# olivier-2018/scene_3Dreconstruction_MVSNet

Measured on AMD Instinct MI355X. Metric: depth maps/sec at N=5 views, 640x512, D=192; achieved HBM GB/s, higher is better.
Workload: dtype f32 (conv0, conv2-4, conv9, conv11: 3xbf16 split operands on the bf16 matrix cores, fp32 accumulate)

## Files before the change

### scene_3dreconstruction_mvsnet_amd/csrc/conv3d_mfma16.hip

```cpp
#include <cstdlib>
#include <cstring>

#include "mvs_internal.h"
#include "storage.h"
#include "mfma16_ops.h"

namespace mvs {

typedef unsigned short u16x8 __attribute__((ext_vector_type(8)));

static inline uint16_t to_bits16(float v, int dt) {
    uint16_t out;
    if (dt == MVS_F16) {
        const _Float16 h = (_Float16)v;
        std::memcpy(&out, &h, 2);
    } else {
        uint32_t u;
        std::memcpy(&u, &v, 4);
        if ((u & 0x7F800000u) == 0x7F800000u && (u & 0x007FFFFFu)) return (uint16_t)((u >> 16) | 0x0040u);
        u += 0x7FFFu + ((u >> 16) & 1u);
        out = (uint16_t)(u >> 16);
    }
    return out;
}

template <int DT>
struct Op16 {
    using T = unsigned short;
    static constexpr int NPC = 1;
    static constexpr bool CLAMP = false;
    struct Stage {
        u32x4 v;
        __device__ __forceinline__ void load(const T* plane, int goff) { v = *reinterpret_cast<const u32x4*>(plane + goff); }
        __device__ __forceinline__ void stage(unsigned short* tile, int tile_elems, int loff, bool inside) const {
            if (loff >= 0) *reinterpret_cast<u32x4*>(tile + loff) = inside ? v : (u32x4){0u, 0u, 0u, 0u};
        }
    };
    template <int N>
    static __device__ __forceinline__ void mac(f32x4& acc, const unsigned short* ap, int tile_elems, const u32x4 (&b)[N], int ks) {
        acc = mfma16<DT>(*reinterpret_cast<const u32x4*>(ap), b[ks], acc);
    }
    struct Skip { float v[8]; };
    static __device__ __forceinline__ void load8(const T* p, size_t idx, Skip& s) { load8_16<DT>(p, idx, s.v); }
    static __device__ __forceinline__ void store8(T* p, size_t idx, f32x4 lo, f32x4 hi) {
        const float v[8] = {lo.x, lo.y, lo.z, lo.w, hi.x, hi.y, hi.z, hi.w};
        store8_16<DT>(p, idx, v);
    }
    static __device__ __forceinline__ void store8(T* p, size_t idx, f32x4 lo, f32x4 hi, const Skip& s) {
        const float v[8] = {lo.x + s.v[0], lo.y + s.v[1], lo.z + s.v[2], lo.w + s.v[3],
                            hi.x + s.v[4], hi.y + s.v[5], hi.z + s.v[6], hi.w + s.v[7]};
        store8_16<DT>(p, idx, v);
    }
};

struct OpSplit {
    using T = float;
    static constexpr int NPC = 3;
    static constexpr bool CLAMP = true;
    struct Stage {
        f32x4 lo, hi;
        __device__ __forceinline__ void load(const T* plane, int goff) {
            lo = *reinterpret_cast<const f32x4*>(plane + goff);
            hi = *reinterpret_cast<const f32x4*>(plane + goff + 4);
        }
        __device__ __forceinline__ void stage(unsigned short* tile, int tile_elems, int loff, bool inside) const {
            const f32x4 z4 = (f32x4){0.f, 0.f, 0.f, 0.f};
            u32x4 p1, p2, p3;
            gs_split8(inside ? lo : z4, inside ? hi : z4, p1, p2, p3);
            *reinterpret_cast<u32x4*>(tile + loff) = p1;
            *reinterpret_cast<u32x4*>(tile + tile_elems + loff) = p2;
            *reinterpret_cast<u32x4*>(tile + 2 * tile_elems + loff) = p3;
        }
    };
    template <int N>
    static __device__ __forceinline__ void mac(f32x4& acc, const unsigned short* ap, int tile_elems, const u32x4 (&b)[N], int ks) {
        constexpr int KS = N / NPC;
        const u32x4 a1 = *reinterpret_cast<const u32x4*>(ap);
        const u32x4 a2 = *reinterpret_cast<const u32x4*>(ap + tile_elems);
        const u32x4 a3 = *reinterpret_cast<const u32x4*>(ap + 2 * tile_elems);
        acc = mfma16<MVS_BF16>(a3, b[ks], acc);
        acc = mfma16<MVS_BF16>(a1, b[2 * KS + ks], acc);
        acc = mfma16<MVS_BF16>(a2, b[KS + ks], acc);
        acc = mfma16<MVS_BF16>(a2, b[ks], acc);
        acc = mfma16<MVS_BF16>(a1, b[KS + ks], acc);
        acc = mfma16<MVS_BF16>(a1, b[ks], acc);
    }
    struct Skip { f32x4 lo, hi; };
    static __device__ __forceinline__ void load8(const T* p, size_t idx, Skip& s) {
        s.lo = *reinterpret_cast<const f32x4*>(p + idx);
        s.hi = *reinterpret_cast<const f32x4*>(p + idx + 4);
    }
    static __device__ __forceinline__ void store8(T* p, size_t idx, f32x4 lo, f32x4 hi) {
        *reinterpret_cast<f32x4*>(p + idx) = lo;
        *reinterpret_cast<f32x4*>(p + idx + 4) = hi;
    }
    static __device__ __forceinline__ void store8(T* p, size_t idx, f32x4 lo, f32x4 hi, const Skip& s) {
        *reinterpret_cast<f32x4*>(p + idx) = lo + s.lo;
        *reinterpret_cast<f32x4*>(p + idx + 4) = hi + s.hi;
    }
};

template <int CIN, int COUT, int S, int BZ, int BY, int BX>
struct ConvG16 {
    static constexpr int NT = COUT / 16;
    static constexpr int MG = 4 / NT;
    static constexpr int MT = BZ * BY * BX;
    static constexpr int MPW = MT / MG;
    static constexpr int NCH = CIN / 8;
    static constexpr int KS = 7;
    static constexpr int VS = 8;
    static constexpr int HZ = (BZ - 1) * S + 3, HY = (2 * BY - 1) * S + 3, HX = (8 * BX - 1) * S + 3;
    static constexpr int HXP = ((HX + 7) / 8 * 8) | 8;
    static constexpr int TILE_ELEMS = HZ * HY * HXP * VS;
    static constexpr int NPIECE = HZ * HY * HX;
    static constexpr int PPT = (NPIECE + 255) / 256;
    static_assert(NT == 1 || NT == 2 || NT == 4, "COUT must be 16, 32 or 64");
    static_assert(MT % MG == 0, "block tile must split evenly over the M-groups");
    static_assert(PPT <= 32, "piece mask is 32 bits");
    static constexpr int tap_off(int tap) {
        const int t = tap > 26 ? 26 : tap;
        return (((t / 9) * HY + (t / 3) % 3) * HXP + t % 3) * VS;
    }
};

template <class Op, int CIN, int COUT, int S, int BZ, int BY, int BX>
__global__ __launch_bounds__(256) void convg16_mfma_kernel(
    const typename Op::T* __restrict__ x,
    const unsigned short* __restrict__ bp,
    const float* __restrict__ bias,
    typename Op::T* __restrict__ y,
    int Di, int Hi, int Wi, int Do, int Ho, int Wo) {
    using G = ConvG16<CIN, COUT, S, BZ, BY, BX>;
    constexpr int OY = 2 * BY, OX = 8 * BX;
    constexpr int RP0 = OX * COUT + 16 * (OX / 8), RP = (RP0 % 32 == 16) ? RP0 : RP0 + 16;
    constexpr int OUT_FLOATS = BZ * OY * RP, NUNIT = BZ * OY * OX * (COUT / 8), UPT = (NUNIT + 255) / 256;
    constexpr int TILE_BYTES = Op::NPC * G::TILE_ELEMS * 2;
    constexpr int LDS_BYTES = TILE_BYTES > OUT_FLOATS * 4 ? TILE_BYTES : OUT_FLOATS * 4;
    __shared__ __attribute__((aligned(16))) unsigned char lds_raw[LDS_BYTES];
    unsigned short* tile = reinterpret_cast<unsigned short*>(lds_raw);
    float* otile = reinterpret_cast<float*>(lds_raw);

    const int tid = threadIdx.x, lane = tid & 63, wave = tid >> 6;
    const int nt = wave % G::NT, mg = wave / G::NT;
    const int nbx = (Wo + 8 * BX - 1) / (8 * BX), nby = (Ho + 2 * BY - 1) / (2 * BY);
    int b = xcd_block();
    const int bx = b % nbx; b /= nbx;
    const int by = b % nby;
    const int bz = b / nby;
    const int ox0 = bx * 8 * BX, oy0 = by * 2 * BY, oz0 = bz * BZ;
    const int ix0 = ox0 * S - 1, iy0 = oy0 * S - 1, iz0 = oz0 * S - 1;
    const size_t Vin = (size_t)Di * Hi * Wi, Vout = (size_t)Do * Ho * Wo;
    constexpr size_t PANEL = (size_t)G::NCH * G::NT * G::KS * 64;

    int goff[G::PPT], loff[G::PPT];
    unsigned inside = 0;
#pragma unroll
    for (int i = 0; i < G::PPT; ++i) {
        const int v = Op::CLAMP ? min(tid + i * 256, G::NPIECE - 1) : tid + i * 256;
        const int hx = v % G::HX, t = v / G::HX;
        const int hy = t % G::HY, hz = t / G::HY;
        const int gz = iz0 + hz, gy = iy0 + hy, gx = ix0 + hx;
        const bool live = Op::CLAMP || v < G::NPIECE;
        const bool ok = live && gz >= 0 && gz < Di && gy >= 0 && gy < Hi && gx >= 0 && gx < Wi;
        goff[i] = ok ? (int)((((size_t)gz * Hi + gy) * Wi + gx) * 8) : 0;
        inside |= ok ? (1u << i) : 0u;
        loff[i] = live ? ((hz * G::HY + hy) * G::HXP + hx) * G::VS : -1;
    }

    const int r = lane & 15, g = lane >> 4;
    const int ry = r >> 3, rx = r & 7;
    int abase[G::MPW];
#pragma unroll
    for (int i = 0; i < G::MPW; ++i) {
        const int t = mg * G::MPW + i;
        const int tx = t % BX, ty = (t / BX) % BY, tz = t / (BX * BY);
        abase[i] = (((tz * S) * G::HY + (2 * ty + ry) * S) * G::HXP + (8 * tx + rx) * S) * G::VS;
    }
    int koff[G::KS];
#pragma unroll
    for (int ks = 0; ks < G::KS; ++ks)
        koff[ks] = g == 0 ? G::tap_off(4 * ks) : g == 1 ? G::tap_off(4 * ks + 1)
                 : g == 2 ? G::tap_off(4 * ks + 2) : G::tap_off(4 * ks + 3);

    f32x4 acc[G::MPW];
#pragma unroll
    for (int i = 0; i < G::MPW; ++i) acc[i] = (f32x4){0.f, 0.f, 0.f, 0.f};
    u32x4 breg[Op::NPC * G::KS];
    typename Op::Stage stg[G::PPT];

    auto load_b = [&](int c) {
        const u32x4* bsrc = reinterpret_cast<const u32x4*>(bp) + ((size_t)(c * G::NT + nt) * G::KS) * 64 + lane;
#pragma unroll
        for (int q = 0; q < Op::NPC; ++q)
#pragma unroll
            for (int ks = 0; ks < G::KS; ++ks) breg[q * G::KS + ks] = bsrc[q * PANEL + ks * 64];
    };
    auto load_a = [&](int c) {
        const typename Op::T* plane = x + (size_t)c * Vin * 8;
#pragma unroll
        for (int i = 0; i < G::PPT; ++i) stg[i].load(plane, goff[i]);
    };
    auto store_a = [&]() {
#pragma unroll
        for (int i = 0; i < G::PPT; ++i) stg[i].stage(tile, G::TILE_ELEMS, loff[i], (inside >> i) & 1u);
    };

    load_b(0);
    load_a(0);
    store_a();
    __syncthreads();

#pragma unroll 1
    for (int c = 0; c < G::NCH; ++c) {
        if (c + 1 < G::NCH) load_a(c + 1);
#pragma unroll
        for (int ks = 0; ks < G::KS; ++ks) {
#pragma unroll
            for (int i = 0; i < G::MPW; ++i) Op::mac(acc[i], tile + abase[i] + koff[ks], G::TILE_ELEMS, breg, ks);
        }
        if (c + 1 < G::NCH) {
            load_b(c + 1);
            __syncthreads();
            store_a();
            __syncthreads();
        }
    }

    const int n = lane & 15, co = 16 * nt + n;
    const float bv = bias[co];
    __syncthreads();
#pragma unroll
    for (int i = 0; i < G::MPW; ++i) {
        const int t = mg * G::MPW + i;
        const int tx = t % BX, ty = (t / BX) % BY, tz = t / (BX * BY);
#pragma unroll
        for (int e = 0; e < 4; ++e) {
            const int m = 4 * (lane >> 4) + e;
            const int oy = 2 * ty + (m >> 3), ox = 8 * tx + (m & 7);
            otile[(tz * OY + oy) * RP + ox * COUT + (ox >> 3) * 16 + co] = relu(acc[i][e] + bv);
        }
    }
    __syncthreads();
#pragma unroll
    for (int j = 0; j < UPT; ++j) {
        const int u = tid + j * 256;
        const int ox = u % OX;
        int t = u / OX;
        const int oy = t % OY; t /= OY;
        const int ozl = t % BZ, pl = t / BZ;
        const int gz = oz0 + ozl, gy = oy0 + oy, gx = ox0 + ox;
        if (u < NUNIT && gz < Do && gy < Ho && gx < Wo) {
            const float* src = otile + (ozl * OY + oy) * RP + ox * COUT + (ox >> 3) * 16 + pl * 8;
            const f32x4 lo = *reinterpret_cast<const f32x4*>(src), hi = *reinterpret_cast<const f32x4*>(src + 4);
            Op::store8(y, ((size_t)pl * Vout + ((size_t)gz * Ho + gy) * Wo + gx) * 8, lo, hi);
        }
    }
}

template <class Op, int CIN, int COUT, int S, int BZ, int BY, int BX>
static int run_convg16(const void* x, void* y, const unsigned short* bp, const float* bias, int Di, int Hi,
                       int Wi, hipStream_t s) {
    using T = typename Op::T;
    const int Do = (Di - 1) / S + 1, Ho = (Hi - 1) / S + 1, Wo = (Wi - 1) / S + 1;
    if ((size_t)Di * Hi * Wi * 8 >= ((size_t)1 << 31))
        return fail(MVS_ERR_BAD_SHAPE, "convg16_mfma: plane exceeds 31-bit offsets");
    const int nb = ((Wo + 8 * BX - 1) / (8 * BX)) * ((Ho + 2 * BY - 1) / (2 * BY)) * ((Do + BZ - 1) / BZ);
    convg16_mfma_kernel<Op, CIN, COUT, S, BZ, BY, BX><<<nb, 256, 0, s>>>(static_cast<const T*>(x), bp, bias,
                                                                         static_cast<T*>(y), Di, Hi, Wi, Do, Ho, Wo);
    return check_hip(hipGetLastError(), "convg16_mfma launch");
}

static bool tile_fills_chip(int Di, int Hi, int Wi, int S, int BZ, int BY, int BX) {
    const int force = options().deep_tiles;
    if (force >= 0) return force != 0;
    const int cus = device_cus();
    const int Do = (Di - 1) / S + 1, Ho = (Hi - 1) / S + 1, Wo = (Wi - 1) / S + 1;
    const long nb = (long)((Wo + 8 * BX - 1) / (8 * BX)) * ((Ho + 2 * BY - 1) / (2 * BY)) * ((Do + BZ - 1) / BZ);
    return 2 * nb >= 3 * (long)cus;
}

template <int DT>
static int launch_convg16_dt(int layer, const void* x, void* y, const unsigned short* bp, const float* bias,
                             int Di, int Hi, int Wi, hipStream_t s) {
    switch (layer) {
        case 1: return run_convg16<Op16<DT>, 8, 16, 2, 2, 2, 2>(x, y, bp, bias, Di, Hi, Wi, s);
        case 2: return run_convg16<Op16<DT>, 16, 16, 1, 2, 4, 2>(x, y, bp, bias, Di, Hi, Wi, s);
        case 3: return run_convg16<Op16<DT>, 16, 32, 2, 4, 1, 1>(x, y, bp, bias, Di, Hi, Wi, s);
        case 4:
            if (tile_fills_chip(Di, Hi, Wi, 1, 4, 2, 1)) return run_convg16<Op16<DT>, 32, 32, 1, 4, 2, 1>(x, y, bp, bias, Di, Hi, Wi, s);
            return run_convg16<Op16<DT>, 32, 32, 1, 1, 2, 2>(x, y, bp, bias, Di, Hi, Wi, s);
        case 5:
            if (tile_fills_chip(Di, Hi, Wi, 2, 2, 1, 1)) return run_convg16<Op16<DT>, 32, 64, 2, 2, 1, 1>(x, y, bp, bias, Di, Hi, Wi, s);
            return run_convg16<Op16<DT>, 32, 64, 2, 1, 1, 1>(x, y, bp, bias, Di, Hi, Wi, s);
        case 6:
            if (tile_fills_chip(Di, Hi, Wi, 1, 4, 1, 1)) return run_convg16<Op16<DT>, 64, 64, 1, 4, 1, 1>(x, y, bp, bias, Di, Hi, Wi, s);
            return run_convg16<Op16<DT>, 64, 64, 1, 1, 1, 1>(x, y, bp, bias, Di, Hi, Wi, s);
        default: return fail(MVS_ERR_BAD_SHAPE, "convg16_mfma: layer %d not covered", layer);
    }
}

void pack_convg16_weights(const float* wfold, int cin, int cout, int dt, unsigned short* bp) {
    const int nch = cin / 8, nt = cout / 16;
    for (int c = 0; c < nch; ++c)
        for (int t = 0; t < nt; ++t)
            for (int ks = 0; ks < 7; ++ks)
                for (int lane = 0; lane < 64; ++lane)
                    for (int j = 0; j < 8; ++j) {
                        const int g = lane >> 4, n = lane & 15;
                        const int tap = 4 * ks + g, ci = 8 * c + j, co = 16 * t + n;
                        const float v = tap < 27 ? wfold[((size_t)tap * cin + ci) * cout + co] : 0.0f;
                        bp[((((size_t)c * nt + t) * 7 + ks) * 64 + lane) * 8 + j] = to_bits16(v, dt);
                    }
}

namespace c16 {
constexpr int TZ = 2, TY = 8, TX = 32;
constexpr int HZ = TZ + 2, HY = TY + 2, HX = TX + 2;
constexpr int VS = 8;
constexpr int TILE_ELEMS = HZ * HY * HX * VS;
constexpr int NPIECE = HZ * HY * HX;
constexpr int PPT = (NPIECE + 255) / 256;
constexpr int KS = 9;
}

template <int DT>
__global__ __launch_bounds__(256) void conv0p16_mfma_kernel(
    const void* __restrict__ x,
    const unsigned short* __restrict__ bp,
    const float* __restrict__ bias,
    void* __restrict__ y,
    int D, int H, int W) {
    using namespace c16;
    __shared__ __attribute__((aligned(16))) unsigned short tile[TILE_ELEMS];
    const unsigned short* xs = static_cast<const unsigned short*>(x);

    const int tid = threadIdx.x, lane = tid & 63, wave = tid >> 6;
    const int nbx = (W + TX - 1) / TX, nby = (H + TY - 1) / TY;
    int b = blockIdx.x;
    const int bx = b % nbx; b /= nbx;
    const int by = b % nby;
    const int bz = b / nby;
    const int x0 = bx * TX, y0 = by * TY, z0 = bz * TZ;
    const size_t V = (size_t)D * H * W;

    int goff[PPT], loff[PPT];
    unsigned inside = 0;
#pragma unroll
    for (int i = 0; i < PPT; ++i) {
        const int v = tid + i * 256;
        const int hx = v % HX, t = v / HX;
        const int hy = t % HY, hz = t / HY;
        const int gz = z0 + hz - 1, gy = y0 + hy - 1, gx = x0 + hx - 1;
        const bool ok = v < NPIECE && gz >= 0 && gz < D && gy >= 0 && gy < H && gx >= 0 && gx < W;
        goff[i] = ok ? (int)((((size_t)gz * H + gy) * W + gx) * 8) : 0;
        inside |= ok ? (1u << i) : 0u;
        loff[i] = (v < NPIECE) ? v * VS : -1;
    }

    const int r = lane & 15, g = lane >> 4;
    const int zt = wave >> 1, yt0 = 4 * (wave & 1);
    const unsigned short* abase = tile + ((zt * HY + yt0) * HX + 2 * r + g) * VS;

    f32x4 acc[4];
#pragma unroll
    for (int i = 0; i < 4; ++i) acc[i] = (f32x4){0.f, 0.f, 0.f, 0.f};
    u32x4 breg[KS];
    u32x4 stg[PPT];

#define MVS_LOAD_B(C)                                                                         \
    {                                                                                         \
        const u32x4* bsrc = reinterpret_cast<const u32x4*>(bp) + (size_t)(C) * KS * 64 + lane; \
        _Pragma("unroll") for (int ks = 0; ks < KS; ++ks) breg[ks] = bsrc[ks * 64];           \
    }
#define MVS_LOAD_A(C)                                                                         \
    {                                                                                         \
        const unsigned short* plane = xs + (size_t)(C) * V * 8;                               \
        _Pragma("unroll") for (int i = 0; i < PPT; ++i)                                       \
// ... 297 lines not shown
    unsigned short* strip = strips + wave * G::STRIP * G::NT;
    const int sm = lane >> 5, sv = (lane >> 1) & 15, sh = lane & 1;
    const bool s_have = sm < G::MPW;
    const int st_t = G::MPW * wave + (s_have ? sm : 0);
    const int sgy = oy0 + 2 * (st_t / (G::TX / 8)) + (sv >> 3), sgx = ox0 + 8 * (st_t % (G::TX / 8)) + (sv & 7);
    const bool st_ok = s_have && sgy < Ho && sgx < Wo;
    const size_t Vout8 = (size_t)Do * Ho * Wo * 8;
    const unsigned st_off = (unsigned)(((size_t)sh * Vout8 + ((size_t)sgy * Wo + sgx) * 8) * 2);
    const unsigned zstep_b = (unsigned)((size_t)Ho * Wo * 8 * 2), nt_b = (unsigned)(2 * Vout8 * 2);
    const __amdgpu_buffer_rsrc_t yrs = __builtin_amdgcn_make_buffer_rsrc(y, (short)0, (int)(unsigned)((COUT / 8) * Vout8 * 2), 0x00020000);

    u32x4 w[3][S][G::PPT];
    {
        u32x4 t0[G::PPT], t1[G::PPT], t2[G::PPT];
        load_plane(S * za - 1, t0);
        load_plane(S * za, t1);
        load_plane(S * za + 1, t2);
#pragma unroll
        for (int q = 0; q < S; ++q) load_plane(S * za + 2 + q, w[0][q]);
#pragma unroll
        for (int q = 0; q < S; ++q) load_plane(S * (za + 1) + 2 + q, w[1][q]);
        store_plane(S * za - 1, t0);
        store_plane(S * za, t1);
        store_plane(S * za + 1, t2);
    }
    __syncthreads();

    auto step = [&](int zo, u32x4 (&cur)[S][G::PPT], u32x4 (&nx)[S][G::PPT]) {
#pragma unroll
        for (int q = 0; q < S; ++q) load_plane(S * (zo + 2) + 2 + q, nx[q]);
        int sb[3];
#pragma unroll
        for (int kz = 0; kz < 3; ++kz) sb[kz] = slot_of(S * zo - 1 + kz);
        f32x4 acc[G::MPW][G::NT];
#pragma unroll
        for (int i = 0; i < G::MPW; ++i)
#pragma unroll
            for (int nt = 0; nt < G::NT; ++nt) acc[i][nt] = (f32x4){0.f, 0.f, 0.f, 0.f};
#pragma unroll
        for (int ks = 0; ks < 7; ++ks) {
            const int sl = (kzl[ks] == 0 ? sb[0] : kzl[ks] == 1 ? sb[1] : sb[2]) + kin[ks];
#pragma unroll
            for (int c = 0; c < G::NCH; ++c)
#pragma unroll
                for (int i = 0; i < G::MPW; ++i) {
                    const u32x4 a = *reinterpret_cast<const u32x4*>(ring + sl + c * G::CHS + mt_off[i]);
#pragma unroll
                    for (int nt = 0; nt < G::NT; ++nt) acc[i][nt] = mfma16<DT>(a, breg[c][nt][ks], acc[i][nt]);
                }
        }
#pragma unroll
        for (int nt = 0; nt < G::NT; ++nt)
#pragma unroll
            for (int i = 0; i < G::MPW; ++i)
#pragma unroll
                for (int e = 0; e < 4; ++e) {
                    const float v = relu(acc[i][nt][e] + bv[nt]);
                    unsigned short bits;
                    if (DT == MVS_F16) { const _Float16 hv = (_Float16)v; bits = __builtin_bit_cast(unsigned short, hv); }
                    else { const __bf16 hv = (__bf16)v; bits = __builtin_bit_cast(unsigned short, hv); }
                    strip[nt * G::STRIP + (i * 16 + 4 * g + e) * 16 + n] = bits;
                }
        __builtin_amdgcn_wave_barrier();
#pragma unroll
        for (int nt = 0; nt < G::NT; ++nt) {
            const u16x8 o = *reinterpret_cast<const u16x8*>(strip + nt * G::STRIP + ((s_have ? sm : 0) * 16 + sv) * 16 + sh * 8);
            __builtin_amdgcn_raw_buffer_store_b128(__builtin_bit_cast(u32x4, o), yrs,
                                                   (int)((st_ok && zo < zb) ? st_off + (unsigned)nt * nt_b + (unsigned)zo * zstep_b : 0xFFFFFFF0u), 0, 0);
        }
        __builtin_amdgcn_wave_barrier();
#pragma unroll
        for (int q = 0; q < S; ++q) store_plane(S * zo + 2 + q, cur[q]);
        __syncthreads();
    };
#pragma unroll 1
    for (int zo = za; zo < zb; zo += 3) {
        step(zo, w[0], w[2]);
        step(zo + 1, w[1], w[0]);
        step(zo + 2, w[2], w[1]);
    }
}

template <int DT, int CIN, int COUT, int S>
static int run_convz16(const void* x, void* y, const unsigned short* bp, const float* bias, int Di, int Hi, int Wi,
                       int Do, int Ho, int Wo, int cus, hipStream_t s) {
    using G = ConvZ16<CIN, COUT, S>;
    const int nbx = (Wo + G::TX - 1) / G::TX, nby = (Ho + G::TY - 1) / G::TY, ncol = nbx * nby;
    int best = 1;
    double best_eff = 0.0;
    for (int nz = 1; nz <= (Do + 3) / 4; ++nz) {
        const int zc = (Do + nz - 1) / nz, nzc = (Do + zc - 1) / zc;
        const long nb = (long)ncol * nzc;
        const double eff = (double)nb / (double)(((nb + cus - 1) / cus) * cus) * zc / (zc + 2.5);
        if (eff > best_eff + 1e-9) { best_eff = eff; best = nz; }
    }
    const int ZC = (Do + best - 1) / best, nzc = (Do + ZC - 1) / ZC;
    convz16_mfma_kernel<DT, CIN, COUT, S><<<ncol * nzc, G::THREADS, 0, s>>>(x, bp, bias, y, Di, Hi, Wi, Do, Ho, Wo, ZC, nbx, nby);
    return check_hip(hipGetLastError(), "convz16_mfma launch");
}

template <int DT>
static int try_convz16(int layer, const void* x, void* y, const unsigned short* bp, const float* bias, int Di, int Hi,
                       int Wi, hipStream_t s, bool* taken) {
    *taken = false;
    const int zm = options().convz16;
    if (zm == 0 || layer < 1 || layer > 3) return MVS_OK;
    const int S = layer == 2 ? 1 : 2, cout = layer == 3 ? 32 : 16;
    const int Do = (Di - 1) / S + 1, Ho = (Hi - 1) / S + 1, Wo = (Wi - 1) / S + 1;
    const int cus = device_cus();
    const int tx = S == 1 ? 32 : 16;
    const long ncol = (long)((Wo + tx - 1) / tx) * ((Ho + 7) / 8);
    if ((size_t)Do * Ho * Wo * cout * 2 >= ((size_t)1 << 32) - 64 || Do < 4) return MVS_OK;
    if (zm != 1 && ncol * (Do / 8) * 4 < (long)cus * 3) return MVS_OK;
    if (zm != 1 && (layer == 3 || (layer == 2 && ncol * (Do / 8) < (long)cus * 3))) return MVS_OK;
    *taken = true;
    switch (layer) {
        case 1: return run_convz16<DT, 8, 16, 2>(x, y, bp, bias, Di, Hi, Wi, Do, Ho, Wo, cus, s);
        case 2: return run_convz16<DT, 16, 16, 1>(x, y, bp, bias, Di, Hi, Wi, Do, Ho, Wo, cus, s);
        default: return run_convz16<DT, 16, 32, 2>(x, y, bp, bias, Di, Hi, Wi, Do, Ho, Wo, cus, s);
    }
}

void pack_conv0p16_weights(const float* wfold, int dt, unsigned short* bp) {
    for (int c = 0; c < 4; ++c)
        for (int ks = 0; ks < 9; ++ks)
            for (int lane = 0; lane < 64; ++lane)
                for (int j = 0; j < 8; ++j) {
                    const int g = lane >> 4, n = lane & 15;
                    const int kz = ks / 3, ky = ks % 3, jj = n >> 3, co = n & 7;
                    const int kx = g - jj, ci = 8 * c + j;
                    float v = 0.0f;
                    if (kx >= 0 && kx <= 2) v = wfold[((size_t)(kz * 9 + ky * 3 + kx) * 32 + ci) * 8 + co];
                    bp[(((size_t)c * 9 + ks) * 64 + lane) * 8 + j] = to_bits16(v, dt);
                }
}


template <int CIN, int COUT, int BZ, int BY, int BX>
struct DeconvG16 {
    static constexpr int NTT = 2 * COUT / 16;
    static constexpr int MG = 4 / NTT;
    static constexpr int MT = BZ * BY * BX;
    static constexpr int MPW = MT / MG;
    static constexpr int NCH = CIN / 8;
    static constexpr int KS = 5;
    static constexpr int VS = 8;
    static constexpr int HZ = BZ + 1, HY = 2 * BY + 1, HX = 8 * BX + 1;
    static constexpr int HXP = ((HX + 7) / 8 * 8) | 8;
    static constexpr int TILE_ELEMS = HZ * HY * HXP * VS;
    static constexpr int NPIECE = HZ * HY * HX;
    static constexpr int PPT = (NPIECE + 255) / 256;
    static_assert(NTT == 1 || NTT == 2 || NTT == 4, "COUT must be 8, 16 or 32");
    static_assert(MT % MG == 0, "block tile must split evenly over the M-groups");
};

template <class Op, int CIN, int COUT, int BZ, int BY, int BX>
__global__ __launch_bounds__(256) void deconvg16_mfma_kernel(
    const typename Op::T* __restrict__ x,
    const unsigned short* __restrict__ bp,
    const float* __restrict__ bias,
    const typename Op::T* __restrict__ skip,
    typename Op::T* __restrict__ y, int Di, int Hi, int Wi) {
    using G = DeconvG16<CIN, COUT, BZ, BY, BX>;
    constexpr int OY = 4 * BY, OX = 16 * BX;
    constexpr int RP0 = OX * COUT + 16 * (OX / 8), RP = (RP0 % 32 == 16) ? RP0 : RP0 + 16;
    constexpr int OUT_FLOATS = BZ * OY * RP, NUNIT = BZ * OY * OX * (COUT / 8), UPT = (NUNIT + 255) / 256;
    constexpr int TILE_BYTES = Op::NPC * G::TILE_ELEMS * 2;
    constexpr int LDS_BYTES = TILE_BYTES > OUT_FLOATS * 4 ? TILE_BYTES : OUT_FLOATS * 4;
    __shared__ __attribute__((aligned(16))) unsigned char lds_raw[LDS_BYTES];
    unsigned short* tile = reinterpret_cast<unsigned short*>(lds_raw);
    float* otile = reinterpret_cast<float*>(lds_raw);

    const int tid = threadIdx.x, lane = tid & 63, wave = tid >> 6;
    const int nt = wave % G::NTT, mg = wave / G::NTT;
    const int nbx = (Wi + 8 * BX - 1) / (8 * BX), nby = (Hi + 2 * BY - 1) / (2 * BY);
    int b = xcd_block();
    const int bx = b % nbx; b /= nbx;
    const int by = b % nby;
    const int bz = b / nby;
    const int ix0 = bx * 8 * BX, iy0 = by * 2 * BY, iz0 = bz * BZ;
    const int Ho = 2 * Hi, Wo = 2 * Wi;
    const size_t Vin = (size_t)Di * Hi * Wi, Vout = Vin * 8;
    constexpr size_t PANEL = (size_t)G::NCH * G::NTT * G::KS * 64;

    int goff[G::PPT], loff[G::PPT];
    unsigned inside = 0;
#pragma unroll
    for (int i = 0; i < G::PPT; ++i) {
        const int v = Op::CLAMP ? min(tid + i * 256, G::NPIECE - 1) : tid + i * 256;
        const int hx = v % G::HX, t = v / G::HX;
        const int hy = t % G::HY, hz = t / G::HY;
        const int gz = iz0 + hz, gy = iy0 + hy, gx = ix0 + hx;
        const bool live = Op::CLAMP || v < G::NPIECE;
        const bool ok = live && gz < Di && gy < Hi && gx < Wi;
        goff[i] = ok ? (int)((((size_t)gz * Hi + gy) * Wi + gx) * 8) : 0;
        inside |= ok ? (1u << i) : 0u;
        loff[i] = live ? ((hz * G::HY + hy) * G::HXP + hx) * G::VS : -1;
    }

    const int r = lane & 15, g = lane >> 4;
    const int ry = r >> 3, rx = r & 7;
    int abase[G::MPW];
#pragma unroll
    for (int i = 0; i < G::MPW; ++i) {
        const int t = mg * G::MPW + i;
        const int tx = t % BX, ty = (t / BX) % BY, tz = t / (BX * BY);
        abase[i] = ((tz * G::HY + 2 * ty + ry) * G::HXP + 8 * tx + rx + (g & 1)) * G::VS;
    }
    int koff[G::KS];
#pragma unroll
    for (int ks = 0; ks < G::KS; ++ks) {
        const Deconv16Tap t0 = deconv16_tap(ks, 0), t1 = deconv16_tap(ks, 1);
        koff[ks] = (g >> 1) ? (t1.dz * G::HY + t1.dy) * G::HXP * G::VS : (t0.dz * G::HY + t0.dy) * G::HXP * G::VS;
    }

    f32x4 acc[4][G::MPW];
#pragma unroll
    for (int c = 0; c < 4; ++c)
#pragma unroll
        for (int i = 0; i < G::MPW; ++i) acc[c][i] = (f32x4){0.f, 0.f, 0.f, 0.f};
    u32x4 breg[Op::NPC * G::KS];
    typename Op::Stage stg[G::PPT];

    auto load_b = [&](int c) {
        const u32x4* bsrc = reinterpret_cast<const u32x4*>(bp) + ((size_t)(c * G::NTT + nt) * G::KS) * 64 + lane;
#pragma unroll
        for (int q = 0; q < Op::NPC; ++q)
#pragma unroll
            for (int ks = 0; ks < G::KS; ++ks) breg[q * G::KS + ks] = bsrc[q * PANEL + ks * 64];
    };
    auto load_a = [&](int c) {
        const typename Op::T* plane = x + (size_t)c * Vin * 8;
#pragma unroll
        for (int i = 0; i < G::PPT; ++i) stg[i].load(plane, goff[i]);
    };
    auto store_a = [&]() {
#pragma unroll
        for (int i = 0; i < G::PPT; ++i) stg[i].stage(tile, G::TILE_ELEMS, loff[i], (inside >> i) & 1u);
    };

    load_b(0);
    load_a(0);
    store_a();
    __syncthreads();

#pragma unroll 1
    for (int c = 0; c < G::NCH; ++c) {
        if (c + 1 < G::NCH) load_a(c + 1);
#pragma unroll
        for (int ks = 0; ks < G::KS; ++ks) {
            const int cls = deconv16_tap(ks, 0).cls;
#pragma unroll
            for (int i = 0; i < G::MPW; ++i)
                Op::mac(acc[cls][i], tile + abase[i] + koff[ks], G::TILE_ELEMS, breg, ks);
        }
        if (c + 1 < G::NCH) {
            load_b(c + 1);
            __syncthreads();
            store_a();
            __syncthreads();
        }
    }

    const int Do = 2 * Di;
    const int nn = 16 * nt + (lane & 15);
    const int px = nn / COUT, co = nn % COUT;
    const float bv = bias[co];
#pragma unroll
    for (int pz = 0; pz < 2; ++pz) {
        size_t uo[UPT];
        int usrc[UPT];
        typename Op::Skip sk[UPT];
#pragma unroll
        for (int j = 0; j < UPT; ++j) {
            const int u = tid + j * 256;
            const int ox = u % OX;
            int t = u / OX;
            const int oy = t % OY; t /= OY;
            const int ozl = t % BZ, pl = t / BZ;
            const int gz = 2 * (iz0 + ozl) + pz, gy = 2 * iy0 + oy, gx = 2 * ix0 + ox;
            const bool ok = u < NUNIT && gz < Do && gy < Ho && gx < Wo;
            usrc[j] = ok ? (ozl * OY + oy) * RP + ox * COUT + (ox >> 3) * 16 + pl * 8 : -1;
            uo[j] = ok ? ((size_t)pl * Vout + ((size_t)gz * Ho + gy) * Wo + gx) * 8 : 0;
            Op::load8(skip, uo[j], sk[j]);
        }
        __syncthreads();
#pragma unroll
        for (int i = 0; i < G::MPW; ++i) {
            const int t = mg * G::MPW + i;
            const int tx = t % BX, ty = (t / BX) % BY, tz = t / (BX * BY);
#pragma unroll
            for (int e = 0; e < 4; ++e) {
                const int m = 4 * (lane >> 4) + e;
                const int ly = 2 * ty + (m >> 3), lx = 8 * tx + (m & 7);
                const int ox = 2 * lx + px;
#pragma unroll
                for (int py = 0; py < 2; ++py)
                    otile[(tz * OY + 2 * ly + py) * RP + ox * COUT + (ox >> 3) * 16 + co] =
                        relu(acc[2 * pz + py][i][e] + bv);
            }
        }
        __syncthreads();
#pragma unroll
        for (int j = 0; j < UPT; ++j) {
            if (usrc[j] < 0) continue;
            const float* src = otile + usrc[j];
            const f32x4 lo = *reinterpret_cast<const f32x4*>(src), hi = *reinterpret_cast<const f32x4*>(src + 4);
            Op::store8(y, uo[j], lo, hi, sk[j]);
        }
    }
}

template <class Op, int CIN, int COUT, int BZ, int BY, int BX>
static int run_deconvg16(const void* x, const void* skip, void* y, const unsigned short* bp,
                         const float* bias, int Di, int Hi, int Wi, hipStream_t s) {
    using T = typename Op::T;
    if ((size_t)Di * Hi * Wi * 8 >= ((size_t)1 << 31))
        return fail(MVS_ERR_BAD_SHAPE, "deconvg16_mfma: plane exceeds 31-bit offsets");
    const int nb = ((Wi + 8 * BX - 1) / (8 * BX)) * ((Hi + 2 * BY - 1) / (2 * BY)) * ((Di + BZ - 1) / BZ);
    deconvg16_mfma_kernel<Op, CIN, COUT, BZ, BY, BX><<<nb, 256, 0, s>>>(static_cast<const T*>(x), bp, bias,
                                                                        static_cast<const T*>(skip),
                                                                        static_cast<T*>(y), Di, Hi, Wi);
    return check_hip(hipGetLastError(), "deconvg16_mfma launch");
}

void pack_deconvg16_weights(const float* wfold, int cin, int cout, int dt, unsigned short* bp) {
    const int nch = cin / 8, ntt = 2 * cout / 16;
    for (int c = 0; c < nch; ++c)
        for (int t = 0; t < ntt; ++t)
            for (int ks = 0; ks < 5; ++ks)
                for (int lane = 0; lane < 64; ++lane)
                    for (int j = 0; j < 8; ++j) {
                        const int g = lane >> 4, n = lane & 15, dx = g & 1;
                        const Deconv16Tap tp = deconv16_tap(ks, g >> 1);
                        const int ci = 8 * c + j;
                        const int nn = 16 * t + n, px = nn / cout, co = nn % cout;
                        const int kx = px == 0 ? (dx == 0 ? 1 : -1) : (dx == 0 ? 2 : 0);
                        const float v = (!tp.valid || kx < 0)
                                            ? 0.0f
                                            : wfold[((size_t)(tp.kz * 9 + tp.ky * 3 + kx) * cin + ci) * cout + co];
                        bp[((((size_t)c * ntt + t) * 5 + ks) * 64 + lane) * 8 + j] = to_bits16(v, dt);
                    }
}

template <int DT>
static int launch_layer16_dt(int layer, const void* x, const void* skip, void* y, const unsigned short* bp,
                             const float* bias, int Di, int Hi, int Wi, hipStream_t s) {
    if (layer == 0) {
        using namespace c16;
        if ((size_t)Di * Hi * Wi * 8 >= ((size_t)1 << 31))
            return fail(MVS_ERR_BAD_SHAPE, "conv0p16_mfma: plane exceeds 31-bit offsets");
        const int zmarch = options().conv0z16;
        const int ncol = ((Wi + c0z::TX - 1) / c0z::TX) * ((Hi + c0z::TY - 1) / c0z::TY);
        const int cus = device_cus();
        if (zmarch != 0 && Di >= 8 && (size_t)Di * Hi * Wi * 16 < ((size_t)1 << 32) - 64 &&
            (zmarch == 1 || (size_t)ncol * (Di / 8) >= (size_t)cus / 2)) {
            int best = 1;
            double best_eff = 0.0;
            for (int nz = 1; nz <= Di / 8; ++nz) {
                const int zc = (Di + nz - 1) / nz, nzc = (Di + zc - 1) / zc;
                const long nb = (long)ncol * nzc;
                const long slots = (long)cus * (8 / c0z::TY);
                const double eff = (double)nb / (double)(((nb + slots - 1) / slots) * slots) * zc / (zc + 2.0);
                if (eff > best_eff + 1e-9) { best_eff = eff; best = nz; }
            }
            const int ZC = (Di + best - 1) / best, nzc = (Di + ZC - 1) / ZC;
            conv0z16_mfma_kernel<DT><<<ncol * nzc, c0z::THREADS, 0, s>>>(x, bp, bias, y, Di, Hi, Wi, ZC,
                                                                          (Wi + c0z::TX - 1) / c0z::TX,
                                                                          (Hi + c0z::TY - 1) / c0z::TY);
            return check_hip(hipGetLastError(), "conv0z16_mfma launch");
        }
        const int nb = ((Wi + TX - 1) / TX) * ((Hi + TY - 1) / TY) * ((Di + TZ - 1) / TZ);
        conv0p16_mfma_kernel<DT><<<nb, 256, 0, s>>>(x, bp, bias, y, Di, Hi, Wi);
        return check_hip(hipGetLastError(), "conv0p16_mfma launch");
    }
    if (layer <= 3) {
        bool taken = false;
        const int st = try_convz16<DT>(layer, x, y, bp, bias, Di, Hi, Wi, s, &taken);
        if (taken) return st;
    }
    if (layer <= 6) return launch_convg16_dt<DT>(layer, x, y, bp, bias, Di, Hi, Wi, s);
    switch (layer) {
        case 7:
            if (tile_fills_chip(Di, Hi, Wi, 1, 2, 1, 1)) return run_deconvg16<Op16<DT>, 64, 32, 2, 1, 1>(x, skip, y, bp, bias, Di, Hi, Wi, s);
            return run_deconvg16<Op16<DT>, 64, 32, 1, 1, 1>(x, skip, y, bp, bias, Di, Hi, Wi, s);
        case 8:
            if (tile_fills_chip(Di, Hi, Wi, 1, 4, 2, 1)) return run_deconvg16<Op16<DT>, 32, 16, 4, 2, 1>(x, skip, y, bp, bias, Di, Hi, Wi, s);
            return run_deconvg16<Op16<DT>, 32, 16, 1, 4, 1>(x, skip, y, bp, bias, Di, Hi, Wi, s);
        case 9: return run_deconvg16<Op16<DT>, 16, 8, 1, 4, 2>(x, skip, y, bp, bias, Di, Hi, Wi, s);
        default: return fail(MVS_ERR_BAD_SHAPE, "mfma16: layer %d not covered", layer);
    }
}

int launch_layer_mfma16(int layer, const void* x, const void* skip, void* y, const void* panel,
                        const float* bias, int Di, int Hi, int Wi, int dtype, hipStream_t s) {
    const unsigned short* bp = static_cast<const unsigned short*>(panel);
    if (dtype == MVS_F16) return launch_layer16_dt<MVS_F16>(layer, x, skip, y, bp, bias, Di, Hi, Wi, s);
    if (dtype == MVS_BF16) return launch_layer16_dt<MVS_BF16>(layer, x, skip, y, bp, bias, Di, Hi, Wi, s);
    return fail(MVS_ERR_BAD_DTYPE, "mfma16 kernels need fp16 or bf16 storage (dtype %d)", dtype);
}

bool split_layer_covers(int layer) {
    const int deconv = options().split_deconv;
    return (layer >= 2 && layer <= 4) || (layer == 7 && (deconv & 1)) || (layer == 8 && (deconv & 2));
}
int launch_layer_split(int layer, const void* x, const void* skip, void* y, const void* panel, const float* bias,
                       int Di, int Hi, int Wi, hipStream_t s) {
    const unsigned short* bp = static_cast<const unsigned short*>(panel);
    switch (layer) {
        case 2: return run_convg16<OpSplit, 16, 16, 1, 2, 4, 2>(x, y, bp, bias, Di, Hi, Wi, s);
        case 3: return run_convg16<OpSplit, 16, 32, 2, 2, 2, 1>(x, y, bp, bias, Di, Hi, Wi, s);
        case 4: return run_convg16<OpSplit, 32, 32, 1, 4, 2, 1>(x, y, bp, bias, Di, Hi, Wi, s);
        case 7: return run_deconvg16<OpSplit, 64, 32, 1, 1, 1>(x, skip, y, bp, bias, Di, Hi, Wi, s);
// ... 40 lines not shown
```

Measured before the change: 1518.

## Interleave per-tap weight prefetch with MFMAs in split-precision conv and deconv kernels

For the 3xbf16 split path, the next channel chunk's weights are now loaded one tap at a time, right after each tap's MFMAs. Scheduling barriers pin that order, so weight loads overlap compute instead of arriving as one burst before the LDS restage. Address math is restructured: the wave index goes to a scalar register via readfirstlane, and the per-lane base is folded into the tap offsets so per-tile offsets become compile-time constants. The launch bounds ask for 3 waves per SIMD when CIN=16, which limits register use and may cause spills.

```diff
diff --git a/scene_3dreconstruction_mvsnet_amd/csrc/conv3d_mfma16.hip b/scene_3dreconstruction_mvsnet_amd/csrc/conv3d_mfma16.hip
--- a/scene_3dreconstruction_mvsnet_amd/csrc/conv3d_mfma16.hip
+++ b/scene_3dreconstruction_mvsnet_amd/csrc/conv3d_mfma16.hip
@@ -1,5 +1,6 @@
 #include <cstdlib>
 #include <cstring>
+#include <type_traits>
 
 #include "mvs_internal.h"
 #include "storage.h"
@@ -24,10 +25,12 @@
     return out;
 }
 
+constexpr int kSchedPin = 0x106;
 template <int DT>
 struct Op16 {
     using T = unsigned short;
     static constexpr int NPC = 1;
+    static constexpr bool STEPWISE = false;
     static constexpr bool CLAMP = false;
     struct Stage {
         u32x4 v;
@@ -56,6 +59,7 @@
 struct OpSplit {
     using T = float;
     static constexpr int NPC = 3;
+    static constexpr bool STEPWISE = true;
     static constexpr bool CLAMP = true;
     struct Stage {
         f32x4 lo, hi;
@@ -121,10 +125,17 @@
         const int t = tap > 26 ? 26 : tap;
         return (((t / 9) * HY + (t / 3) % 3) * HXP + t % 3) * VS;
     }
+    static constexpr int mt_off(int t) {
+        return ((((t / (BX * BY)) * S) * HY + 2 * ((t / BX) % BY) * S) * HXP + 8 * (t % BX) * S) * VS;
+    }
+    static constexpr bool MT_SPLITS = BX % MPW == 0 || (MPW % BX == 0 && BY % (MPW / BX) == 0) || MPW % (BX * BY) == 0;
 };
 
+template <class Op, int CIN>
+constexpr int convg16_waves() { return (Op::STEPWISE && CIN == 16) ? 3 : 1; }
+
 template <class Op, int CIN, int COUT, int S, int BZ, int BY, int BX>
-__global__ __launch_bounds__(256) void convg16_mfma_kernel(
+__global__ __launch_bounds__(256, (convg16_waves<Op, CIN>())) void convg16_mfma_kernel(
     const typename Op::T* __restrict__ x,
     const unsigned short* __restrict__ bp,
     const float* __restrict__ bias,
@@ -140,7 +151,8 @@
     unsigned short* tile = reinterpret_cast<unsigned short*>(lds_raw);
     float* otile = reinterpret_cast<float*>(lds_raw);
 
-    const int tid = threadIdx.x, lane = tid & 63, wave = tid >> 6;
+    const int tid = threadIdx.x, lane = tid & 63;
+    const int wave = Op::STEPWISE ? __builtin_amdgcn_readfirstlane(tid >> 6) : tid >> 6;
     const int nt = wave % G::NT, mg = wave / G::NT;
     const int nbx = (Wo + 8 * BX - 1) / (8 * BX), nby = (Ho + 2 * BY - 1) / (2 * BY);
     int b = xcd_block();
@@ -169,18 +181,28 @@
 
     const int r = lane & 15, g = lane >> 4;
     const int ry = r >> 3, rx = r & 7;
-    int abase[G::MPW];
-#pragma unroll
-    for (int i = 0; i < G::MPW; ++i) {
-        const int t = mg * G::MPW + i;
-        const int tx = t % BX, ty = (t / BX) % BY, tz = t / (BX * BY);
-        abase[i] = (((tz * S) * G::HY + (2 * ty + ry) * S) * G::HXP + (8 * tx + rx) * S) * G::VS;
-    }
-    int koff[G::KS];
-#pragma unroll
-    for (int ks = 0; ks < G::KS; ++ks)
-        koff[ks] = g == 0 ? G::tap_off(4 * ks) : g == 1 ? G::tap_off(4 * ks + 1)
-                 : g == 2 ? G::tap_off(4 * ks + 2) : G::tap_off(4 * ks + 3);
+    int aoff[G::MPW], koff[G::KS];
+    if constexpr (Op::STEPWISE) {
+        const int mt0 = G::mt_off(mg * G::MPW);
+        const int abase = mt0 + ((ry * S) * G::HXP + rx * S) * G::VS;
+#pragma unroll
+        for (int i = 0; i < G::MPW; ++i) aoff[i] = G::MT_SPLITS ? G::mt_off(i) : G::mt_off(mg * G::MPW + i) - mt0;
+#pragma unroll
+        for (int ks = 0; ks < G::KS; ++ks)
+            koff[ks] = abase + (g == 0 ? G::tap_off(4 * ks) : g == 1 ? G::tap_off(4 * ks + 1)
+                              : g == 2 ? G::tap_off(4 * ks + 2) : G::tap_off(4 * ks + 3));
+    } else {
+#pragma unroll
+        for (int i = 0; i < G::MPW; ++i) {
+            const int t = mg * G::MPW + i;
+            const int tx = t % BX, ty = (t / BX) % BY, tz = t / (BX * BY);
+            aoff[i] = (((tz * S) * G::HY + (2 * ty + ry) * S) * G::HXP + (8 * tx + rx) * S) * G::VS;
+        }
+#pragma unroll
+        for (int ks = 0; ks < G::KS; ++ks)
+            koff[ks] = g == 0 ? G::tap_off(4 * ks) : g == 1 ? G::tap_off(4 * ks + 1)
+                     : g == 2 ? G::tap_off(4 * ks + 2) : G::tap_off(4 * ks + 3);
+    }
 
     f32x4 acc[G::MPW];
 #pragma unroll
@@ -188,6 +210,21 @@
     u32x4 breg[Op::NPC * G::KS];
     typename Op::Stage stg[G::PPT];
 
+    auto load_b_step = [&](int c, int ks) {
+        const u32x4* bsrc = reinterpret_cast<const u32x4*>(bp) + ((size_t)(c * G::NT + nt) * G::KS + ks) * 64 + lane;
+#pragma unroll
+        for (int q = 0; q < Op::NPC; ++q) breg[q * G::KS + ks] = bsrc[q * PANEL];
+    };
+    auto load_a = [&](int c) {
+        const typename Op::T* plane = x + (size_t)c * Vin * 8;
+#pragma unroll
+        for (int i = 0; i < G::PPT; ++i) stg[i].load(plane, goff[i]);
+    };
+    auto store_a = [&]() {
+#pragma unroll
+        for (int i = 0; i < G::PPT; ++i) stg[i].stage(tile, G::TILE_ELEMS, loff[i], (inside >> i) & 1u);
+    };
+
     auto load_b = [&](int c) {
         const u32x4* bsrc = reinterpret_cast<const u32x4*>(bp) + ((size_t)(c * G::NT + nt) * G::KS) * 64 + lane;
 #pragma unroll
@@ -195,34 +232,59 @@
 #pragma unroll
             for (int ks = 0; ks < G::KS; ++ks) breg[q * G::KS + ks] = bsrc[q * PANEL + ks * 64];
     };
-    auto load_a = [&](int c) {
-        const typename Op::T* plane = x + (size_t)c * Vin * 8;
-#pragma unroll
-        for (int i = 0; i < G::PPT; ++i) stg[i].load(plane, goff[i]);
-    };
-    auto store_a = [&]() {
-#pragma unroll
-        for (int i = 0; i < G::PPT; ++i) stg[i].stage(tile, G::TILE_ELEMS, loff[i], (inside >> i) & 1u);
-    };
-
-    load_b(0);
-    load_a(0);
-    store_a();
-    __syncthreads();
-
+
+    if constexpr (Op::STEPWISE) {
+        load_a(0);
+#pragma unroll
+        for (int ks = 0; ks < G::KS; ++ks) load_b_step(0, ks);
+        store_a();
+        __syncthreads();
+
+        auto chunk = [&](int c, auto more) {
+            constexpr bool MORE = decltype(more)::value;
+            if (MORE) {
+                load_a(c + 1);
+                __builtin_amdgcn_sched_barrier(kSchedPin);
+            }
+#pragma unroll
+            for (int ks = 0; ks < G::KS; ++ks) {
+#pragma unroll
+                for (int i = 0; i < G::MPW; ++i) Op::mac(acc[i], tile + aoff[i] + koff[ks], G::TILE_ELEMS, breg, ks);
+                if (MORE) {
+                    load_b_step(c + 1, ks);
+                    __builtin_amdgcn_sched_barrier(kSchedPin);
+                }
+            }
+            if (MORE) {
+                __builtin_amdgcn_sched_barrier(0);
+                __syncthreads();
+                store_a();
+                __syncthreads();
+            }
+        };
 #pragma unroll 1
-    for (int c = 0; c < G::NCH; ++c) {
-        if (c + 1 < G::NCH) load_a(c + 1);
-#pragma unroll
-        for (int ks = 0; ks < G::KS; ++ks) {
-#pragma unroll
-            for (int i = 0; i < G::MPW; ++i) Op::mac(acc[i], tile + abase[i] + koff[ks], G::TILE_ELEMS, breg, ks);
-        }
-        if (c + 1 < G::NCH) {
-            load_b(c + 1);
-            __syncthreads();
-            store_a();
-            __syncthreads();
+        for (int c = 0; c < G::NCH - 1; ++c) chunk(c, std::true_type{});
+        chunk(G::NCH - 1, std::false_type{});
+    } else {
+        load_b(0);
+        load_a(0);
+        store_a();
+        __syncthreads();
+
+#pragma unroll 1
+        for (int c = 0; c < G::NCH; ++c) {
+            if (c + 1 < G::NCH) load_a(c + 1);
+#pragma unroll
+            for (int ks = 0; ks < G::KS; ++ks) {
+#pragma unroll
+                for (int i = 0; i < G::MPW; ++i) Op::mac(acc[i], tile + aoff[i] + koff[ks], G::TILE_ELEMS, breg, ks);
+            }
+            if (c + 1 < G::NCH) {
+                load_b(c + 1);
+                __syncthreads();
+                store_a();
+                __syncthreads();
+            }
         }
     }
 
@@ -826,6 +888,8 @@
     static constexpr int PPT = (NPIECE + 255) / 256;
     static_assert(NTT == 1 || NTT == 2 || NTT == 4, "COUT must be 8, 16 or 32");
     static_assert(MT % MG == 0, "block tile must split evenly over the M-groups");
+    static constexpr int mt_off(int t) { return (((t / (BX * BY)) * HY + 2 * ((t / BX) % BY)) * HXP + 8 * (t % BX)) * VS; }
+    static constexpr bool MT_SPLITS = BX % MPW == 0 || (MPW % BX == 0 && BY % (MPW / BX) == 0) || MPW % (BX * BY) == 0;
 };
 
 template <class Op, int CIN, int COUT, int BZ, int BY, int BX>
@@ -845,7 +909,8 @@
     unsigned short* tile = reinterpret_cast<unsigned short*>(lds_raw);
     float* otile = reinterpret_cast<float*>(lds_raw);
 
-    const int tid = threadIdx.x, lane = tid & 63, wave = tid >> 6;
+    const int tid = threadIdx.x, lane = tid & 63;
+    const int wave = Op::STEPWISE ? __builtin_amdgcn_readfirstlane(tid >> 6) : tid >> 6;
     const int nt = wave % G::NTT, mg = wave / G::NTT;
     const int nbx = (Wi + 8 * BX - 1) / (8 * BX), nby = (Hi + 2 * BY - 1) / (2 * BY);
     int b = xcd_block();
@@ -874,18 +939,29 @@
 
     const int r = lane & 15, g = lane >> 4;
     const int ry = r >> 3, rx = r & 7;
-    int abase[G::MPW];
-#pragma unroll
-    for (int i = 0; i < G::MPW; ++i) {
-        const int t = mg * G::MPW + i;
-        const int tx = t % BX, ty = (t / BX) % BY, tz = t / (BX * BY);
-        abase[i] = ((tz * G::HY + 2 * ty + ry) * G::HXP + 8 * tx + rx + (g & 1)) * G::VS;
-    }
-    int koff[G::KS];
-#pragma unroll
-    for (int ks = 0; ks < G::KS; ++ks) {
-        const Deconv16Tap t0 = deconv16_tap(ks, 0), t1 = deconv16_tap(ks, 1);
-        koff[ks] = (g >> 1) ? (t1.dz * G::HY + t1.dy) * G::HXP * G::VS : (t0.dz * G::HY + t0.dy) * G::HXP * G::VS;
+    int aoff[G::MPW], koff[G::KS];
+    if constexpr (Op::STEPWISE) {
+        const int mt0 = G::mt_off(mg * G::MPW);
+        const int abase = mt0 + (ry * G::HXP + rx + (g & 1)) * G::VS;
+#pragma unroll
+        for (int i = 0; i < G::MPW; ++i) aoff[i] = G::MT_SPLITS ? G::mt_off(i) : G::mt_off(mg * G::MPW + i) - mt0;
+#pragma unroll
+        for (int ks = 0; ks < G::KS; ++ks) {
+            const Deconv16Tap t0 = deconv16_tap(ks, 0), t1 = deconv16_tap(ks, 1);
+            koff[ks] = abase + ((g >> 1) ? (t1.dz * G::HY + t1.dy) * G::HXP * G::VS : (t0.dz * G::HY + t0.dy) * G::HXP * G::VS);
+        }
+    } else {
+#pragma unroll
+        for (int i = 0; i < G::MPW; ++i) {
+            const int t = mg * G::MPW + i;
+            const int tx = t % BX, ty = (t / BX) % BY, tz = t / (BX * BY);
+            aoff[i] = ((tz * G::HY + 2 * ty + ry) * G::HXP + 8 * tx + rx + (g & 1)) * G::VS;
+        }
+#pragma unroll
+        for (int ks = 0; ks < G::KS; ++ks) {
+            const Deconv16Tap t0 = deconv16_tap(ks, 0), t1 = deconv16_tap(ks, 1);
+            koff[ks] = (g >> 1) ? (t1.dz * G::HY + t1.dy) * G::HXP * G::VS : (t0.dz * G::HY + t0.dy) * G::HXP * G::VS;
+        }
     }
 
     f32x4 acc[4][G::MPW];
@@ -896,6 +972,21 @@
     u32x4 breg[Op::NPC * G::KS];
     typename Op::Stage stg[G::PPT];
 
+    auto load_b_step = [&](int c, int ks) {
+        const u32x4* bsrc = reinterpret_cast<const u32x4*>(bp) + ((size_t)(c * G::NTT + nt) * G::KS + ks) * 64 + lane;
+#pragma unroll
+        for (int q = 0; q < Op::NPC; ++q) breg[q * G::KS + ks] = bsrc[q * PANEL];
+    };
+    auto load_a = [&](int c) {
+        const typename Op::T* plane = x + (size_t)c * Vin * 8;
+#pragma unroll
+        for (int i = 0; i < G::PPT; ++i) stg[i].load(plane, goff[i]);
+    };
+    auto store_a = [&]() {
+#pragma unroll
+        for (int i = 0; i < G::PPT; ++i) stg[i].stage(tile, G::TILE_ELEMS, loff[i], (inside >> i) & 1u);
+    };
+
     auto load_b = [&](int c) {
         const u32x4* bsrc = reinterpret_cast<const u32x4*>(bp) + ((size_t)(c * G::NTT + nt) * G::KS) * 64 + lane;
 #pragma unroll
@@ -903,36 +994,61 @@
 #pragma unroll
             for (int ks = 0; ks < G::KS; ++ks) breg[q * G::KS + ks] = bsrc[q * PANEL + ks * 64];
     };
-    auto load_a = [&](int c) {
-        const typename Op::T* plane = x + (size_t)c * Vin * 8;
-#pragma unroll
-        for (int i = 0; i < G::PPT; ++i) stg[i].load(plane, goff[i]);
-    };
-    auto store_a = [&]() {
-#pragma unroll
-        for (int i = 0; i < G::PPT; ++i) stg[i].stage(tile, G::TILE_ELEMS, loff[i], (inside >> i) & 1u);
-    };
-
-    load_b(0);
-    load_a(0);
-    store_a();
-    __syncthreads();
-
+
+    if constexpr (Op::STEPWISE) {
+        load_a(0);
+#pragma unroll
+        for (int ks = 0; ks < G::KS; ++ks) load_b_step(0, ks);
+        store_a();
+        __syncthreads();
+
+        auto chunk = [&](int c, auto more) {
+            constexpr bool MORE = decltype(more)::value;
+            if (MORE) {
+                load_a(c + 1);
+                __builtin_amdgcn_sched_barrier(kSchedPin);
+            }
+#pragma unroll
+            for (int ks = 0; ks < G::KS; ++ks) {
+                const int cls = deconv16_tap(ks, 0).cls;
+#pragma unroll
+                for (int i = 0; i < G::MPW; ++i) Op::mac(acc[cls][i], tile + aoff[i] + koff[ks], G::TILE_ELEMS, breg, ks);
+                if (MORE) {
+                    load_b_step(c + 1, ks);
+                    __builtin_amdgcn_sched_barrier(kSchedPin);
+                }
+            }
+            if (MORE) {
+                __builtin_amdgcn_sched_barrier(0);
+                __syncthreads();
+                store_a();
+                __syncthreads();
+            }
+        };
 #pragma unroll 1
-    for (int c = 0; c < G::NCH; ++c) {
-        if (c + 1 < G::NCH) load_a(c + 1);
-#pragma unroll
-        for (int ks = 0; ks < G::KS; ++ks) {
-            const int cls = deconv16_tap(ks, 0).cls;
-#pragma unroll
-            for (int i = 0; i < G::MPW; ++i)
-                Op::mac(acc[cls][i], tile + abase[i] + koff[ks], G::TILE_ELEMS, breg, ks);
-        }
-        if (c + 1 < G::NCH) {
-            load_b(c + 1);
-            __syncthreads();
-            store_a();
-            __syncthreads();
+        for (int c = 0; c < G::NCH - 1; ++c) chunk(c, std::true_type{});
+        chunk(G::NCH - 1, std::false_type{});
+    } else {
+        load_b(0);
+        load_a(0);
+        store_a();
+        __syncthreads();
+
+#pragma unroll 1
+        for (int c = 0; c < G::NCH; ++c) {
+            if (c + 1 < G::NCH) load_a(c + 1);
+#pragma unroll
+            for (int ks = 0; ks < G::KS; ++ks) {
+                const int cls = deconv16_tap(ks, 0).cls;
+#pragma unroll
+                for (int i = 0; i < G::MPW; ++i) Op::mac(acc[cls][i], tile + aoff[i] + koff[ks], G::TILE_ELEMS, breg, ks);
+            }
+            if (c + 1 < G::NCH) {
+                load_b(c + 1);
+                __syncthreads();
+                store_a();
+                __syncthreads();
+            }
         }
     }
 
```

Result: faster. 1539 (median of 6 runs) (+1.4%).
